# orottier/web-audio-api-rs

Measured on AMD Instinct MI355X. Metric: render quanta/sec (48kHz, 128-frame), higher is better.
Workload: dtype f64

## Files before the change

### web-audio-api-rs_amd/csrc/waa_hrtf_fft.hip

```cpp
#include <hip/hip_runtime.h>

#include "waa_hrtf_fft.hpp"
#include "waa_internal.hpp"

namespace waa {
namespace {
using namespace hrtffft;
constexpr int WAVES = 4;

__device__ __forceinline__ void wsync() {
  __builtin_amdgcn_sched_barrier(0);
  __builtin_amdgcn_wave_barrier();
  __builtin_amdgcn_sched_barrier(0);
}

template <bool EXACTZ>
__global__ __launch_bounds__(WAVES * 64) __attribute__((amdgpu_waves_per_eu(1, 1))) void hrtf_fft_kernel(const HrtfDesc d) {
  extern __shared__ __attribute__((aligned(16))) float lds_raw[];
  const ldsp tab = (ldsp)lds_raw;
  const int lane = threadIdx.x & 63, wv = (int)__builtin_amdgcn_readfirstlane(threadIdx.x >> 6);
  const int g = lane >> 4, t = lane & 15;
  const ldsp ex = tab + PARTS * TAB_SLOTS + (wv * 4 + g) * XSLOTS;
  const uint64_t gid = ((uint64_t)blockIdx.x * WAVES + wv) * 4 + g;
  const uint32_t inst = (uint32_t)(gid / d.n_seg_pad), seg = (uint32_t)(gid % d.n_seg_pad);
  const bool alive = inst < d.n_inst && seg < d.n_seg;
  const uint32_t row = d.rows > 1 && inst < d.n_inst ? inst : 0u;
  {
    const f4v* src = reinterpret_cast<const f4v*>(d.fft_tables + (uint64_t)row * (PARTS * TAB_SLOTS * 2));
    __attribute__((address_space(3))) f4v* dst = (__attribute__((address_space(3))) f4v*)tab;
    for (int i = threadIdx.x; i < PARTS * TAB_SLOTS / 2; i += WAVES * 64) dst[i] = load_global_f4(reinterpret_cast<const float*>(src + i));
  }
  __syncthreads();
  const int32_t* prev = d.prev + (uint64_t)(alive ? inst : 0) * d.prev_stride;
  const uint8_t* code = d.in_code + (uint64_t)(alive ? inst : 0) * d.code_stride;
  const int q_lo = (int)(d.q0 + seg * d.seg_len);
  const int q_hi = (int)((uint64_t)q_lo + d.seg_len < d.q1 ? q_lo + d.seg_len : d.q1);
  int ph[HEADS];
#pragma unroll
  for (int k = 0; k < HEADS; k++) ph[k] = -1;
  if (q_lo > 0) {
    int base = q_lo - 1, p1 = -1;
    bool searching = alive && q_lo < (int)d.q1;
    while (__builtin_amdgcn_ballot_w64(searching) != 0) {
      const int qq = base - t;
      const int32_t l = (searching && qq >= 0) ? load_global(prev + qq) : LINK_SKIP;
      const uint64_t hit = __builtin_amdgcn_ballot_w64(l != LINK_SKIP) >> (g * 16) & 0xffffull;
      if (searching) {
        if (hit) {
          p1 = base - __builtin_ctzll(hit);
          searching = false;
        } else {
          base -= 16;
          if (base < 0) searching = false;
        }
      }
    }
    int p = p1;
#pragma unroll
    for (int k = HEADS - 1; k >= 0; k--) {
      ph[k] = p;
      if (p >= 0) {
        const int32_t l = load_global(prev + p);
        p = l >= 0 ? l : -1;
      }
    }
  }
  HLane L;
  load_tw(reinterpret_cast<const c2v*>(d.tw256), t, L.tws);
  lane_reset_if(L, true);
  const float* src = d.in.base + (uint64_t)(alive ? inst : 0) * d.in.inst_stride;
  float* dst = d.out.base + (uint64_t)(alive ? inst : 0) * d.out.inst_stride;
  const float gain = load_global(&d.table[row].gain);
  int jmax_l = 0, jmax_r = 0, lastnz = -8192;
  if constexpr (EXACTZ) {
    jmax_l = load_global(d.jmax + 2 * row);
    jmax_r = load_global(d.jmax + 2 * row + 1);
  }
  const int n_it = (int)d.seg_len + HEADS;
  auto quantum_of = [&](int it) { return it < HEADS ? (it == 0 ? ph[0] : it == 1 ? ph[1] : it == 2 ? ph[2] : ph[3]) : q_lo + it - HEADS; };
  auto valid_at = [&](int it, int q) { return alive && it < n_it && q >= 0 && (it < HEADS || q < q_hi); };
  const float* safe = d.tw256;
  float xn0[8], xn1[8];
  int zpos[8];
  int32_t link_n;
  uint32_t code_n;
  auto request = [&](int q, bool procn, uint32_t c) __attribute__((always_inline)) {
    const bool live = procn && !(c & CODE_SILENT);
    const float* p0 = live ? src + (uint64_t)q * RQ + t : safe + t;
    const float* p1c = live && (c & 63u) >= 2 ? p0 + d.in.ch_stride : safe + t;
#pragma unroll
    for (int j = 0; j < 8; j++) {
      xn0[j] = load_global(p0 + 16 * j);
      xn1[j] = load_global(p1c + 16 * j);
    }
  };
  {
    const int q0 = quantum_of(0);
    const bool v = valid_at(0, q0);
    link_n = v ? load_global(prev + q0) : LINK_SKIP;
    code_n = v ? (uint32_t)load_global(code + q0) : (uint32_t)CODE_SILENT;
    request(q0, link_n != LINK_SKIP, code_n);
  }
#pragma unroll 1
  for (int it = 0; it < n_it; it++) {
    const int q = quantum_of(it);
    const int32_t link = link_n;
    const uint32_t c = code_n;
    const bool proc = link != LINK_SKIP;
    const bool store = alive && it >= HEADS && q < q_hi;
    const int qn = quantum_of(it + 1);
    {
      const bool v = valid_at(it + 1, qn);
      link_n = v ? load_global(prev + qn) : LINK_SKIP;
      code_n = v ? (uint32_t)load_global(code + qn) : (uint32_t)CODE_SILENT;
    }
    lane_reset_if(L, proc && link == LINK_FRESH);
    if constexpr (EXACTZ) lastnz = proc && link == LINK_FRESH ? -8192 : lastnz;
    int tofs = 0;
    asm volatile("" : "+s"(tofs));
    const ldsp tabq = tab + tofs;
    {
      const bool live = proc && !(c & CODE_SILENT), st2 = (c & 63u) >= 2;
      float x[8];
#pragma unroll
      for (int j = 0; j < 8; j++) {
        const float m = st2 ? 0.5f * (xn0[j] + xn1[j]) : xn0[j];
        x[j] = live ? m : 0.f;
      }
      if constexpr (EXACTZ) {
        int run_last = lastnz;
#pragma unroll
        for (int j = 0; j < 8; j++) {
          const uint64_t bal = __builtin_amdgcn_ballot_w64(x[j] != 0.f);
          const uint32_t rm = (uint32_t)(bal >> (g * 16)) & 0xffffu;
          const uint32_t below = rm & ((2u << t) - 1u);
          zpos[j] = below ? 16 * j + (31 - __builtin_clz(below)) : run_last;
          run_last = rm ? 16 * j + (31 - __builtin_clz(rm)) : run_last;
        }
        const int nxt = run_last - 128 < -8192 ? -8192 : run_last - 128;
        lastnz = proc ? nxt : lastnz;
      }
      ph_in(L, x);
    }
    xwrite(L.a, ex, t);
    wsync();
    xread(L.a, ex, t);
    wsync();
    ph_spec(L, tabq, t, proc);
    request(qn, link_n != LINK_SKIP, code_n);
    xwrite(L.Y, ex, t);
    wsync();
    xread(L.Y, ex, t);
    wsync();
    c2v o[8];
    ph_out(L, proc, o);
    {
      const float corr = (c & 63u) >= 2 ? 2.f : 1.f;
      float* p0 = store ? dst + (uint64_t)q * RQ + t : d.trash + lane;
      float* p1c = store ? p0 + d.out.ch_stride : d.trash + lane;
#pragma unroll
      for (int j = 0; j < 8; j++) {
        float ol = proc ? o[j].x * gain * corr : 0.f, orr = proc ? o[j].y * gain * corr : 0.f;
        if constexpr (EXACTZ) {
          const int back = 16 * j + t - zpos[j];
          ol = back > jmax_l ? 0.f : ol;
          orr = back > jmax_r ? 0.f : orr;
        }
        store_global(p0 + (store ? 16 * j : 0), ol);
        store_global(p1c + (store ? 16 * j : 0), orr);
      }
    }
  }
}
__global__ __launch_bounds__(256) void hrtf_fft_tables_kernel(const float* pairs, uint32_t pair_stride, int taps, const double* cs_sn, float* out) {
  const uint32_t row = blockIdx.x / PARTS, p = blockIdx.x % PARTS;
  const int kp = (int)threadIdx.x;
  const float* pair = pairs + (uint64_t)row * pair_stride;
  double re = 0., im = 0.;
  for (int n = 0; n < 128; n++) {
    const int tap = 128 * (int)p + n;
    if (tap >= taps) break;
    const double hl = (double)pair[(size_t)tap * 2], hr = (double)pair[(size_t)tap * 2 + 1];
    const int e = (kp * n) & 255;
    const double c = cs_sn[e], sn = cs_sn[256 + e];
    re += hl * c - hr * sn;
    im += hl * sn + hr * c;
  }
  const int t = kp & 15, j = kp >> 4;
  const size_t slot = (size_t)t * ROW + (size_t)K16(j);
  float* o = out + (((uint64_t)row * PARTS + p) * TAB_SLOTS + slot) * 2;
  o[0] = (float)(re / 256.);
  o[1] = (float)(im / 256.);
}
}

void launch_hrtf_fft_tables(const float* pairs, uint32_t pair_stride, int taps, uint32_t rows, const double* cs_sn, float* out, void* stream) {
  (void)hipMemsetAsync(out, 0, (size_t)rows * PARTS * TAB_SLOTS * 2 * sizeof(float), (hipStream_t)stream);
  hipLaunchKernelGGL(hrtf_fft_tables_kernel, dim3(rows * PARTS), dim3(256), 0, (hipStream_t)stream, pairs, pair_stride, taps, cs_sn, out);
}

void launch_hrtf_fft(const HrtfDesc& d0, void* stream) {
  HrtfDesc d = d0;
  if (d.q1 == 0) d.q1 = d.n_quanta;
  if (d.q1 <= d.q0) return;
  const uint32_t nq = d.q1 - d.q0;
  if (d.q0 != 0 || d.q1 != d.n_quanta || d.seg_len == 0) {
    const uint32_t fill = (uint32_t)(((uint64_t)d.n_inst * nq + 16383) / 16384);
    d.seg_len = nq < 8 ? nq : (fill > 8 ? (fill < nq ? fill : nq) : 8);
  }
  d.n_seg = (nq + d.seg_len - 1) / d.seg_len;
  d.n_seg_pad = d.rows > 1 ? (d.n_seg + WAVES * 4 - 1) / (WAVES * 4) * (WAVES * 4) : d.n_seg;
  const size_t lds = ((size_t)PARTS * TAB_SLOTS + (size_t)WAVES * 4 * XSLOTS) * 8;
  const uint64_t groups = (uint64_t)d.n_inst * d.n_seg_pad;
  const dim3 grid((unsigned)((groups + WAVES * 4 - 1) / (WAVES * 4))), block(WAVES * 64);
  if (d.jmax)
    hipLaunchKernelGGL(hrtf_fft_kernel<true>, grid, block, lds, (hipStream_t)stream, d);
  else
    hipLaunchKernelGGL(hrtf_fft_kernel<false>, grid, block, lds, (hipStream_t)stream, d);
}

}
```

### web-audio-api-rs_amd/csrc/waa_hrtf_fft.hpp

```cpp
#pragma once
#include "waa_osfft.hpp"

namespace waa {
namespace hrtffft {

using namespace osfft;
constexpr int PARTS = 4;
constexpr int HEADS = PARTS;

struct HLane {
  c2v a[16];
  c2v Y[16];
  c2v Zh[PARTS - 1][16];
  c2v ocar[8];
  Tw tws;
};
F3_FN void lane_reset_if(HLane& L, bool fresh) {
#pragma unroll
  for (int j = 0; j < 8; j++) {
    L.ocar[j].x = fresh ? 0.f : L.ocar[j].x;
    L.ocar[j].y = fresh ? 0.f : L.ocar[j].y;
  }
#pragma unroll
  for (int p = 0; p < PARTS - 1; p++)
#pragma unroll
    for (int s = 0; s < 16; s++) {
      L.Zh[p][s].x = fresh ? 0.f : L.Zh[p][s].x;
      L.Zh[p][s].y = fresh ? 0.f : L.Zh[p][s].y;
    }
}
F3_FN void ph_in(HLane& L, const float (&x)[8]) {
#pragma unroll
  for (int j = 0; j < 8; j++) L.a[j] = c2v{x[j], 0.f};
  pass1_half<false>(L.a, L.tws);
}
F3_FN void ph_spec(HLane& L, cldsp tab, int t, bool proc) {
  pass2<false>(L.a);
#pragma unroll
  for (int h = 0; h < 2; h++) {
#pragma unroll
    for (int p = 0; p < PARTS; p++) {
      c2v w[8];
      tab_read8(w, tab + p * TAB_SLOTS, t, h);
#pragma unroll
      for (int s = 8 * h; s < 8 * h + 8; s += 4) {
        const int o = s - 8 * h;
        if (p == 0)
          cmul4<false>(L.Y[K16(s)], L.Y[K16(s + 1)], L.Y[K16(s + 2)], L.Y[K16(s + 3)], L.a[s], L.a[s + 1], L.a[s + 2], L.a[s + 3], w[o], w[o + 1],
                       w[o + 2], w[o + 3]);
        else
          cmac4(L.Y[K16(s)], L.Y[K16(s + 1)], L.Y[K16(s + 2)], L.Y[K16(s + 3)], L.Zh[p - 1][s], L.Zh[p - 1][s + 1], L.Zh[p - 1][s + 2],
                L.Zh[p - 1][s + 3], w[o], w[o + 1], w[o + 2], w[o + 3]);
      }
    }
  }
#pragma unroll
  for (int s = 0; s < 16; s++) {
#pragma unroll
    for (int p = PARTS - 2; p > 0; p--) {
      L.Zh[p][s].x = proc ? L.Zh[p - 1][s].x : L.Zh[p][s].x;
      L.Zh[p][s].y = proc ? L.Zh[p - 1][s].y : L.Zh[p][s].y;
    }
    L.Zh[0][s].x = proc ? L.a[s].x : L.Zh[0][s].x;
    L.Zh[0][s].y = proc ? L.a[s].y : L.Zh[0][s].y;
  }
  pass1<true>(L.Y, L.tws);
}
F3_FN void ph_out(HLane& L, bool proc, c2v (&o)[8]) {
  pass2<true>(L.Y);
#pragma unroll
  for (int j = 0; j < 8; j++) {
    o[j] = L.Y[K16(j)] + L.ocar[j];
    const c2v nxt = L.Y[K16(j + 8)];
    L.ocar[j].x = proc ? nxt.x : L.ocar[j].x;
    L.ocar[j].y = proc ? nxt.y : L.ocar[j].y;
  }
}

}
}
```

Baseline: 2.952 billion.

## Spill oldest HRTF partition history to LDS to fit two waves per SIMD

```diff
diff --git a/web-audio-api-rs_amd/csrc/waa_hrtf_fft.hip b/web-audio-api-rs_amd/csrc/waa_hrtf_fft.hip
--- a/web-audio-api-rs_amd/csrc/waa_hrtf_fft.hip
+++ b/web-audio-api-rs_amd/csrc/waa_hrtf_fft.hip
@@ -7,6 +7,8 @@
 namespace {
 using namespace hrtffft;
 constexpr int WAVES = 4;
+constexpr int WPS = 2;
+constexpr int LDS_SLOTS = PARTS * TAB_SLOTS + WAVES * 4 * XSLOTS + WAVES * HIST_WAVE_SLOTS;
 
 __device__ __forceinline__ void wsync() {
   __builtin_amdgcn_sched_barrier(0);
@@ -15,12 +17,13 @@
 }
 
 template <bool EXACTZ>
-__global__ __launch_bounds__(WAVES * 64) __attribute__((amdgpu_waves_per_eu(1, 1))) void hrtf_fft_kernel(const HrtfDesc d) {
+__global__ __launch_bounds__(WAVES * 64) __attribute__((amdgpu_waves_per_eu(WPS, WPS))) void hrtf_fft_kernel(const HrtfDesc d) {
   extern __shared__ __attribute__((aligned(16))) float lds_raw[];
   const ldsp tab = (ldsp)lds_raw;
   const int lane = threadIdx.x & 63, wv = (int)__builtin_amdgcn_readfirstlane(threadIdx.x >> 6);
   const int g = lane >> 4, t = lane & 15;
   const ldsp ex = tab + PARTS * TAB_SLOTS + (wv * 4 + g) * XSLOTS;
+  const ldsp hist = tab + PARTS * TAB_SLOTS + WAVES * 4 * XSLOTS + wv * HIST_WAVE_SLOTS + 2 * lane;
   const uint64_t gid = ((uint64_t)blockIdx.x * WAVES + wv) * 4 + g;
   const uint32_t inst = (uint32_t)(gid / d.n_seg_pad), seg = (uint32_t)(gid % d.n_seg_pad);
   const bool alive = inst < d.n_inst && seg < d.n_seg;
@@ -65,9 +68,10 @@
       }
     }
   }
-  HLane L;
-  load_tw(reinterpret_cast<const c2v*>(d.tw256), t, L.tws);
-  lane_reset_if(L, true);
+  HLaneL L;
+  Tw tws;
+  load_tw(reinterpret_cast<const c2v*>(d.tw256), t, tws);
+  lane_reset_if(L, hist, true);
   const float* src = d.in.base + (uint64_t)(alive ? inst : 0) * d.in.inst_stride;
   float* dst = d.out.base + (uint64_t)(alive ? inst : 0) * d.out.inst_stride;
   const float gain = load_global(&d.table[row].gain);
@@ -114,7 +118,7 @@
       link_n = v ? load_global(prev + qn) : LINK_SKIP;
       code_n = v ? (uint32_t)load_global(code + qn) : (uint32_t)CODE_SILENT;
     }
-    lane_reset_if(L, proc && link == LINK_FRESH);
+    lane_reset_if(L, hist, proc && link == LINK_FRESH);
     if constexpr (EXACTZ) lastnz = proc && link == LINK_FRESH ? -8192 : lastnz;
     int tofs = 0;
     asm volatile("" : "+s"(tofs));
@@ -140,13 +144,13 @@
         const int nxt = run_last - 128 < -8192 ? -8192 : run_last - 128;
         lastnz = proc ? nxt : lastnz;
       }
-      ph_in(L, x);
+      ph_in(L, tws, x);
     }
     xwrite(L.a, ex, t);
     wsync();
     xread(L.a, ex, t);
     wsync();
-    ph_spec(L, tabq, t, proc);
+    ph_spec(L, tws, tabq, hist, t, proc);
     request(qn, link_n != LINK_SKIP, code_n);
     xwrite(L.Y, ex, t);
     wsync();
@@ -210,7 +214,9 @@
   }
   d.n_seg = (nq + d.seg_len - 1) / d.seg_len;
   d.n_seg_pad = d.rows > 1 ? (d.n_seg + WAVES * 4 - 1) / (WAVES * 4) * (WAVES * 4) : d.n_seg;
-  const size_t lds = ((size_t)PARTS * TAB_SLOTS + (size_t)WAVES * 4 * XSLOTS) * 8;
+  static_assert(LDS_SLOTS * 8 == 9216 + 16 * 2432 + 16 * 2048 && (LDS_SLOTS * 8 + 1279) / 1280 * 1280 * WPS <= 160 * 1024,
+                "two workgroups of hrtf_fft_kernel per CU");
+  const size_t lds = (size_t)LDS_SLOTS * 8;
   const uint64_t groups = (uint64_t)d.n_inst * d.n_seg_pad;
   const dim3 grid((unsigned)((groups + WAVES * 4 - 1) / (WAVES * 4))), block(WAVES * 64);
   if (d.jmax)
diff --git a/web-audio-api-rs_amd/csrc/waa_hrtf_fft.hpp b/web-audio-api-rs_amd/csrc/waa_hrtf_fft.hpp
--- a/web-audio-api-rs_amd/csrc/waa_hrtf_fft.hpp
+++ b/web-audio-api-rs_amd/csrc/waa_hrtf_fft.hpp
@@ -29,10 +29,93 @@
       L.Zh[p][s].y = fresh ? 0.f : L.Zh[p][s].y;
     }
 }
+constexpr int HIST_LANES = 64;
+constexpr int HIST_WAVE_SLOTS = HIST_LANES * 16;
+struct HLaneL {
+  c2v a[16];
+  c2v Y[16];
+  c2v Zh[PARTS - 2][16];
+  c2v ocar[8];
+};
+F3_FN void hist_read4(c2v (&z)[8], cldsp hist, int h) {
+  const F3_LDS fft3::f4v_* p = (const F3_LDS fft3::f4v_*)hist;
+#pragma unroll
+  for (int j = 0; j < 4; j++) {
+    const fft3::f4v_ v = p[(4 * h + j) * HIST_LANES];
+    z[2 * j] = c2v{v.x, v.y};
+    z[2 * j + 1] = c2v{v.z, v.w};
+  }
+}
+F3_FN void hist_write(ldsp hist, const c2v (&z)[16]) {
+  F3_LDS fft3::f4v_* p = (F3_LDS fft3::f4v_*)hist;
+#pragma unroll
+  for (int j = 0; j < 8; j++) p[j * HIST_LANES] = fft3::f4v_{z[2 * j].x, z[2 * j].y, z[2 * j + 1].x, z[2 * j + 1].y};
+}
+F3_FN void lane_reset_if(HLaneL& L, ldsp hist, bool fresh) {
+#pragma unroll
+  for (int j = 0; j < 8; j++) {
+    L.ocar[j].x = fresh ? 0.f : L.ocar[j].x;
+    L.ocar[j].y = fresh ? 0.f : L.ocar[j].y;
+  }
+#pragma unroll
+  for (int p = 0; p < PARTS - 2; p++)
+#pragma unroll
+    for (int s = 0; s < 16; s++) {
+      L.Zh[p][s].x = fresh ? 0.f : L.Zh[p][s].x;
+      L.Zh[p][s].y = fresh ? 0.f : L.Zh[p][s].y;
+    }
+  if (fresh) {
+    F3_LDS fft3::f4v_* p = (F3_LDS fft3::f4v_*)hist;
+#pragma unroll
+    for (int j = 0; j < 8; j++) p[j * HIST_LANES] = fft3::f4v_{0.f, 0.f, 0.f, 0.f};
+  }
+}
+F3_FN void ph_spec(HLaneL& L, const Tw& tws, cldsp tab, ldsp hist, int t, bool proc) {
+  pass2<false>(L.a);
+#pragma unroll
+  for (int h = 0; h < 2; h++) {
+#pragma unroll
+    for (int p = 0; p < PARTS; p++) {
+      c2v w[8], zo[8];
+      tab_read8(w, tab + p * TAB_SLOTS, t, h);
+      if (p == PARTS - 1) hist_read4(zo, hist, h);
+#pragma unroll
+      for (int s = 8 * h; s < 8 * h + 8; s += 4) {
+        const int o = s - 8 * h;
+        if (p == 0)
+          cmul4<false>(L.Y[K16(s)], L.Y[K16(s + 1)], L.Y[K16(s + 2)], L.Y[K16(s + 3)], L.a[s], L.a[s + 1], L.a[s + 2], L.a[s + 3], w[o], w[o + 1],
+                       w[o + 2], w[o + 3]);
+        else if (p == PARTS - 1)
+          cmac4(L.Y[K16(s)], L.Y[K16(s + 1)], L.Y[K16(s + 2)], L.Y[K16(s + 3)], zo[o], zo[o + 1], zo[o + 2], zo[o + 3], w[o], w[o + 1], w[o + 2],
+                w[o + 3]);
+        else
+          cmac4(L.Y[K16(s)], L.Y[K16(s + 1)], L.Y[K16(s + 2)], L.Y[K16(s + 3)], L.Zh[p - 1][s], L.Zh[p - 1][s + 1], L.Zh[p - 1][s + 2],
+                L.Zh[p - 1][s + 3], w[o], w[o + 1], w[o + 2], w[o + 3]);
+      }
+    }
+  }
+  if (proc) hist_write(hist, L.Zh[PARTS - 3]);
+#pragma unroll
+  for (int s = 0; s < 16; s++) {
+#pragma unroll
+    for (int p = PARTS - 3; p > 0; p--) {
+      L.Zh[p][s].x = proc ? L.Zh[p - 1][s].x : L.Zh[p][s].x;
+      L.Zh[p][s].y = proc ? L.Zh[p - 1][s].y : L.Zh[p][s].y;
+    }
+    L.Zh[0][s].x = proc ? L.a[s].x : L.Zh[0][s].x;
+    L.Zh[0][s].y = proc ? L.a[s].y : L.Zh[0][s].y;
+  }
+  pass1<true>(L.Y, tws);
+}
 F3_FN void ph_in(HLane& L, const float (&x)[8]) {
 #pragma unroll
   for (int j = 0; j < 8; j++) L.a[j] = c2v{x[j], 0.f};
   pass1_half<false>(L.a, L.tws);
+}
+F3_FN void ph_in(HLaneL& L, const Tw& tws, const float (&x)[8]) {
+#pragma unroll
+  for (int j = 0; j < 8; j++) L.a[j] = c2v{x[j], 0.f};
+  pass1_half<false>(L.a, tws);
 }
 F3_FN void ph_spec(HLane& L, cldsp tab, int t, bool proc) {
   pass2<false>(L.a);
@@ -66,7 +149,8 @@
   }
   pass1<true>(L.Y, L.tws);
 }
-F3_FN void ph_out(HLane& L, bool proc, c2v (&o)[8]) {
+template <class LaneT>
+F3_FN void ph_out(LaneT& L, bool proc, c2v (&o)[8]) {
   pass2<true>(L.Y);
 #pragma unroll
   for (int j = 0; j < 8; j++) {
```

Result: no change. 2.942 billion, median of 4 (-0.3%).
